# speechcatcher-asr/speechcatcher

Hardware: AMD Instinct MI355X
Metric: concurrent real-time streams (audio-seconds/s), de_xl dims, 640 ms (10240-sample) chunk steps, beam 10 CTC+attention (higher is better)
Workload: dtype f32

## Files before the change

include/scasr.h:

```cpp
#ifndef SCASR_H
#define SCASR_H

#include <stddef.h>
#include <stdint.h>

#ifdef __cplusplus
extern "C" {
#endif

#define SC_OK 0
#define SC_ERR_ARG (-1)
#define SC_ERR_LAUNCH (-2)
#define SC_ERR_CAPACITY (-3)
#define SC_ERR_INPUT (-4)

#define SC_GEMM_RELU 1
#define SC_GEMM_RESIDUAL 2
#define SC_GEMM_LN_AT_CROWS 8
#define SC_GEMM_NAIVE 4
#define SC_GEMM_SPLIT16 16

#define SC_F_ANY_EOS 1
#define SC_F_BEST_EOS 2
#define SC_F_ALL_EOS 4
// ... 351 lines not shown
int sc_ctc_extend_state(const sc_search *sb , void *stream);
int sc_dec_embed(const sc_search *sb, void *stream);
int sc_kv_rows_to_half(const float *stage, const int32_t *rows, int m, int n_layers, int TCAP, int d2,
                       void *ckv_half, void *stream);
int sc_dec_self_attn(const sc_search *sb, int layer, void *stream);
int sc_dec_cross_attn(const sc_search *sb, int layer, void *stream);
int sc_decoder_layers(const sc_search *sb, void *stream);
#define SC_MAX_VOCAB 8192
int sc_logsoftmax_topk(const sc_search *sb, void *stream);
int sc_ctc_prefix_scan(const sc_search *sb, void *stream);
int sc_ctc_prefix_scan_split(const sc_search *sb, int split_min, void *stream);
int sc_fuse_topw(const sc_search *sb, void *stream);
int sc_beam_prune(const sc_search *sb, void *stream);
int sc_ctc_gather_state(const sc_search *sb, void *stream);
int sc_ctc_gather_state_split(const sc_search *sb, int split_min, void *stream);
int sc_decode_step(const sc_search *sb, void *stream);
int sc_decode_step_ex(const sc_search *sb, int scan_split_min, void *stream);
int sc_dec_layer_fused_supported(int d, int H, int W, int F);
int sc_dec_layer_self(const sc_search *sb, int layer, const float *x_in, float *x_out, const float *ffn_part,
                      int n_ffn_part, void *stream);
int sc_dec_layer_cross(const sc_search *sb, int layer, const float *x_in, float *x_out, void *stream);
int sc_dec_layer_ffn(const sc_search *sb, int layer, const float *x_in, float *x_out, float *ffn_part,
                     int max_part, int *n_part , void *stream);
int sc_dec_layer_stream_supported(int d, int H, int W, int F);
int sc_dec_layer_stream(const sc_search *sb, int layer, const float *x_in, float *x_out, float *xn_out,
                        const float *ffn_part, int n_ffn_part, void *stream);
int sc_dec_layer_ffn_xn(const sc_search *sb, int layer, const float *xn, float *ffn_part, int max_part,
                        int *n_part , void *stream);
int sc_dec_layer_reduce_ln(const sc_search *sb, int layer, const float *x_in, float *x_out, float *xn_out, void *stream);
int sc_dec_output_logits(const sc_search *sb, const float *x_in, float *x_out, const float *ffn_part,
// ... 126 lines not shown
```

speechcatcher_amd/_abi.py:

```python
import ctypes as C
import os
import subprocess
from pathlib import Path

HERE = Path(__file__).resolve().parent
LIB_PATH = HERE / "libscasr.so"
CSRC = HERE / "csrc"

c_float_p = C.POINTER(C.c_float)
c_int_p = C.POINTER(C.c_int32)
c_double_p = C.POINTER(C.c_double)
vp = C.c_void_p


class EncLayer(C.Structure):
    _fields_ = [(n, vp) for n in ("ln1_g", "ln1_b", "wqkv", "bqkv", "wo", "bo",
                                  "ln2_g", "ln2_b", "w1", "b1", "w2", "b2", "w1_p", "w2_p",
                                  "wqkv_p", "wo_p", "w1_h", "w2_h", "wqkv_h", "wo_h", "w1_s", "w2_s",
                                  "wqkv_s", "wo_s")]


class DecLayer(C.Structure):
    _fields_ = [(n, vp) for n in ("ln1_g", "ln1_b", "wqkv", "bqkv", "wo", "bo",
                                  "ln2_g", "ln2_b", "wq", "bq", "wo2", "bo2",
# ... 181 lines not shown
    "sc_relpos_attention": (C.c_int, [vp, vp, vp, vp, vp, C.c_int, C.c_int, C.c_int, C.c_int, vp]),
    "sc_relpos_attention_masked": (C.c_int, [vp, vp, vp, vp, vp, C.c_int, C.c_int, C.c_int, C.c_int, vp, C.c_int, vp]),
    "sc_ctc_extend_state": (C.c_int, [vp, vp]),
    "sc_dec_embed": (C.c_int, [vp, vp]),
    "sc_kv_rows_to_half": (C.c_int, [vp, vp, C.c_int, C.c_int, C.c_int, C.c_int, vp, vp]),
    "sc_dec_self_attn": (C.c_int, [vp, C.c_int, vp]),
    "sc_dec_cross_attn": (C.c_int, [vp, C.c_int, vp]),
    "sc_decoder_layers": (C.c_int, [vp, vp]),
    "sc_logsoftmax_topk": (C.c_int, [vp, vp]),
    "sc_ctc_prefix_scan": (C.c_int, [vp, vp]),
    "sc_fuse_topw": (C.c_int, [vp, vp]),
    "sc_beam_prune": (C.c_int, [vp, vp]),
    "sc_ctc_gather_state": (C.c_int, [vp, vp]),
    "sc_ctc_gather_state_split": (C.c_int, [vp, C.c_int, vp]),
    "sc_decode_step": (C.c_int, [vp, vp]),
    "sc_decode_step_ex": (C.c_int, [vp, C.c_int, vp]),
    "sc_ctc_prefix_scan_split": (C.c_int, [vp, C.c_int, vp]),
    "sc_dec_layer_fused_supported": (C.c_int, [C.c_int, C.c_int, C.c_int, C.c_int]),
    "sc_dec_layer_self": (C.c_int, [vp, C.c_int, vp, vp, vp, C.c_int, vp]),
    "sc_dec_layer_cross": (C.c_int, [vp, C.c_int, vp, vp, vp]),
    "sc_dec_layer_ffn": (C.c_int, [vp, C.c_int, vp, vp, vp, C.c_int, C.POINTER(C.c_int), vp]),
    "sc_dec_output_logits": (C.c_int, [vp, vp, vp, vp, C.c_int, vp]),
    "sc_streams_kv_rows": (C.c_int, [vp]),
    "sc_dec_layer_stream_supported": (C.c_int, [C.c_int, C.c_int, C.c_int, C.c_int]),
    "sc_dec_layer_stream": (C.c_int, [vp, C.c_int, vp, vp, vp, vp, C.c_int, vp]),
    "sc_dec_layer_reduce_ln": (C.c_int, [vp, C.c_int, vp, vp, vp, vp]),
    "sc_dec_layer_ffn_xn": (C.c_int, [vp, C.c_int, vp, vp, C.c_int, C.POINTER(C.c_int), vp]),
    "sc_engine_create": (C.c_int, [C.POINTER(Config), C.POINTER(NamedTensor), C.c_int, C.c_int, C.POINTER(vp)]),
    "sc_engine_load": (C.c_int, [C.c_char_p, C.c_int, C.POINTER(vp)]),
    "sc_engine_config": (C.c_int, [vp, C.POINTER(Config)]),
# ... 125 lines not shown
```

speechcatcher_amd/csrc/search.hip:

```cpp
#include "common.h"
#include "attn.h"
#include <mutex>
#include <unordered_map>

#define CTRL(s, f) sb.ctrl[(s) * 8 + (f)]
#define SC_CTC_T(s) (CTRL(s, SC_C_TCTC) > 0 ? CTRL(s, SC_C_TCTC) : CTRL(s, SC_C_T))

#define YSEQ(pp, s, h) (sb.yseq + (((long)(pp) * sb.S + (s)) * sb.W + (h)) * sb.LCAP)
#define XPOS(pp, s, h) (sb.xpos + (((long)(pp) * sb.S + (s)) * sb.W + (h)) * sb.LCAP)
#define ANC(pp, s) (sb.anc + ((long)(pp) * sb.S + (s)) * sb.LCAP * sb.W)
#define CTCR(pp, s) (sb.ctc_r + ((long)(pp) * sb.S + (s)) * sb.TCAP * 2 * sb.W)
#define CTCRS(pp, s) (sb.ctc_rs + ((long)(pp) * sb.S + (s)) * sb.TCAP * sb.W)

__global__ void ctc_extend_state_kernel(sc_search sb) {
  const int s = blockIdx.x, h = threadIdx.x;
  if (!CTRL(s, SC_C_ACTIVE) || !CTRL(s, SC_C_HAS)) return;
  const int T = CTRL(s, SC_C_T), told = CTRL(s, SC_C_TOLD), nh = CTRL(s, SC_C_NHYP);
  if (h >= nh || told >= T) return;
  float *r = CTCR(CTRL(s, SC_C_CUR), s);
  float *rs = CTCRS(CTRL(s, SC_C_CUR), s);
  const float *x = sb.ctcx + (long)s * sb.TCAP * sb.V;
  const int t0 = told < 1 ? 1 : told;
  float rb = r[((long)(t0 - 1) * 2 + 1) * sb.W + h];
  for (int t = t0; t < T; ++t) {
// ... 474 lines not shown
  else {
    const size_t lds = pow2_keys_bytes(sbp->V);
    const int rc = allow_large_lds(reinterpret_cast<const void *>(&logsoftmax_topk_sort_kernel), lds,
                                   pow2_keys_bytes(SC_MAX_VOCAB), "sc_logsoftmax_topk");
    if (rc != SC_OK) return rc;
    logsoftmax_topk_sort_kernel<<<sbp->S * sbp->W, 256, lds, (hipStream_t)stream>>>(*sbp);
  }
  SC_CHECK_LAUNCH();
  return SC_OK;
}

struct CtcChunkT {
  float4 xc[4], xb[4];
  float pn[16], pb[16];
};
#define SC_CTC_CK 16
__host__ __device__ static inline int ctc_tck(int TCAP) { return (TCAP + SC_CTC_CK - 1) / SC_CTC_CK; }
__device__ __forceinline__ void ctc_frame(float &r_n, float &r_b, float prs, float pb, bool same, float xc, float xb, float &phi) {
  phi = same ? pb : prs;
  const float nr_n = lse2(r_n, phi) + xc;
  const float nr_b = lse2(r_n, r_b) + xb;
  r_n = nr_n;
  r_b = nr_b;
}
__device__ __forceinline__ void ctc_psi_add(float &pm, float &ps, float v) {
  const float d = v - pm;
  const float e = sc_exp_neg(-fabsf(d));
  ps = d > 0.f ? ps * e + 1.f : ps + e;
  pm = sc_max_raw(pm, v);
}
__device__ __forceinline__ bool ctc_scan_is_split(int T, int L, int split_min) {
  const int out_len = L - 1;
  int start = out_len > 1 ? out_len : 1;
  if (start > T) start = T;
  return split_min > 0 && T - start >= split_min;
}
#define CTC_NSEG 32
static inline int ctc_split_min_ok(int TCAP, int split_min) { return ctc_tck(TCAP) >= CTC_NSEG ? split_min : 0; }

__global__ __launch_bounds__(256) void ctc_prefix_scan_colmajor_kernel(sc_search sb, int split_min) {
  const int s = blockIdx.y;
  if (!CTRL(s, SC_C_ACTIVE)) return;
  const int nh = CTRL(s, SC_C_NHYP), K = sb.K, W = sb.W, V = sb.V;
  const int e = blockIdx.x * 256 + threadIdx.x;
  if (e >= nh * K) return;
  const int h = e / K, k = e % K;
  const int T = SC_CTC_T(s), L = CTRL(s, SC_C_L), cur = CTRL(s, SC_C_CUR);
  if (ctc_scan_is_split(T, L, split_min)) return;
  const bool has = CTRL(s, SC_C_HAS);
  const long row = (long)s * W + h;
  const int c = sb.pre_ids[row * K + k];
  const int last = YSEQ(cur, s, h)[L - 1];
  const bool same = (c == last);
  const int tct = sb.tct;
  const float *__restrict__ xcol = sb.ctcxT + ((long)s * V + c) * tct;
  const float *__restrict__ xblk = sb.ctcxT + ((long)s * V + sb.blank) * tct;
  const float *__restrict__ rp = CTCR(cur, s);
  const float *__restrict__ rsp = CTCRS(cur, s);
  float *rn = sb.ctc_rnew + (long)s * ctc_tck(sb.TCAP) * 2 * (W * K);
  const int WK = W * K;
  const int out_len = L - 1;
  int start = out_len > 1 ? out_len : 1;
  if (start > T) start = T;
  for (int j = 0; SC_CTC_CK * j + SC_CTC_CK - 1 < start - 1; ++j) {
    rn[((long)j * 2) * WK + e] = SC_LOGZERO;
    rn[((long)j * 2 + 1) * WK + e] = SC_LOGZERO;
  }
  float r_n = (out_len == 0) ? xcol[0] : SC_LOGZERO;
  float r_b = SC_LOGZERO;
  if (((start - 1) & (SC_CTC_CK - 1)) == SC_CTC_CK - 1) {
    rn[((long)((start - 1) / SC_CTC_CK) * 2) * WK + e] = r_n;
    rn[((long)((start - 1) / SC_CTC_CK) * 2 + 1) * WK + e] = r_b;
  }
  float cum = 0.f;
  if (!has)
    for (int t = 0; t < start; ++t) cum += xblk[t];

  auto fetch = [&](CtcChunkT &q, int tb) {
#pragma unroll
    for (int j = 0; j < 4; ++j) {
      const int t4 = min(tb + 4 * j, tct - 4);
      q.xc[j] = *reinterpret_cast<const float4 *>(xcol + t4);
      q.xb[j] = *reinterpret_cast<const float4 *>(xblk + t4);
    }
    if (has) {
#pragma unroll
      for (int i = 0; i < 16; ++i) {
        int t = tb + i;
        t = t < T ? (t < 1 ? 1 : t) : T - 1;
        q.pn[i] = rsp[(long)(t - 1) * W + h];
        q.pb[i] = rp[((long)(t - 1) * 2 + 1) * W + h];
      }
    }
  };
  float pm = r_n, ps = 1.f;
  auto frame = [&](const CtcChunkT &q, int tb, int i) {
    const int t = tb + i;
    const float4 c4 = q.xc[i >> 2], b4 = q.xb[i >> 2];
    const float xc = (i & 3) == 0 ? c4.x : (i & 3) == 1 ? c4.y : (i & 3) == 2 ? c4.z : c4.w;
    const float xb = (i & 3) == 0 ? b4.x : (i & 3) == 1 ? b4.y : (i & 3) == 2 ? b4.z : b4.w;
    const float prs = has ? q.pn[i] : cum;
    const float pb = has ? q.pb[i] : cum;
    float phi;
    ctc_frame(r_n, r_b, prs, pb, same, xc, xb, phi);
    if ((i & (SC_CTC_CK - 1)) == SC_CTC_CK - 1) {
      rn[((long)(t / SC_CTC_CK) * 2) * WK + e] = r_n;
      rn[((long)(t / SC_CTC_CK) * 2 + 1) * WK + e] = r_b;
    }
    ctc_psi_add(pm, ps, phi + xc);
    if (!has) cum += xb;
  };
  auto advance = [&](const CtcChunkT &q, int tb) {
    if (tb >= start && tb + 16 <= T) {
#pragma unroll
      for (int i = 0; i < 16; ++i) frame(q, tb, i);
    } else {
#pragma unroll
      for (int i = 0; i < 16; ++i)
        if (tb + i >= start && tb + i < T) frame(q, tb, i);
    }
  };
  if (start < T) {
    CtcChunkT qa, qb;
    int tb = start & ~15;
    fetch(qa, tb);
    while (true) {
      if (tb + 16 < T) fetch(qb, tb + 16);
      advance(qa, tb);
      tb += 16;
      if (tb >= T) break;
      if (tb + 16 < T) fetch(qa, tb + 16);
      advance(qb, tb);
      tb += 16;
      if (tb >= T) break;
    }
  }
  float psi = pm + logf(ps);
  const float rsum_last = has ? rsp[(long)(T - 1) * W + h] : cum;
  if (c == sb.eos) psi = rsum_last;
  if (c == sb.blank) psi = SC_LOGZERO;
  sb.psi[row * K + k] = psi;
  if (k == 0) sb.psi_eos[row] = rsum_last;
}

#define CTC_EB (256 / CTC_NSEG)
__global__ __launch_bounds__(256) void ctc_prefix_scan_tpar_kernel(sc_search sb, int split_min) {
  __shared__ float co[8][CTC_NSEG][CTC_EB];
  __shared__ float st0[2][CTC_NSEG][CTC_EB];
  __shared__ float cum0[CTC_NSEG][CTC_EB];
  const int s = blockIdx.y;
  if (!CTRL(s, SC_C_ACTIVE)) return;
// ... 143 lines not shown
  std::lock_guard<std::mutex> lk(g_scan_split_mutex);
  g_scan_split[sbp->ctc_rnew] = eff;
}
static int scan_split_last(const sc_search *sbp) {
  std::lock_guard<std::mutex> lk(g_scan_split_mutex);
  auto it = g_scan_split.find(sbp->ctc_rnew);
  return it == g_scan_split.end() ? -1 : it->second;
}

extern "C" int sc_ctc_prefix_scan_split(const sc_search *sbp, int split_min, void *stream) {
  SC_CHECK_ARG(sbp, "null");
  SC_CHECK_ARG(sbp->ctcxT && sbp->tct >= 4 && sbp->tct % 4 == 0, "the prefix scan needs the column-major table copy (sc_search.ctcxT)");
  split_min = ctc_split_min_ok(sbp->TCAP, split_min);
  scan_split_note(sbp, split_min);
  dim3 grid(cdiv(sbp->W * sbp->K, 256), sbp->S);
  ctc_prefix_scan_colmajor_kernel<<<grid, 256, 0, (hipStream_t)stream>>>(*sbp, split_min);
  if (split_min > 0)
    ctc_prefix_scan_tpar_kernel<<<dim3(cdiv(sbp->W * sbp->K, CTC_EB), sbp->S), 256, 0, (hipStream_t)stream>>>(*sbp, split_min);
  SC_CHECK_LAUNCH();
  return SC_OK;
}

extern "C" int sc_ctc_prefix_scan(const sc_search *sbp, void *stream) { return sc_ctc_prefix_scan_split(sbp, 0, stream); }

__device__ __forceinline__ float sort_key_value(unsigned long long c) {
  unsigned u = (unsigned)(c >> 32);
  u = (u & 0x80000000u) ? (u & 0x7FFFFFFFu) : ~u;
  return __uint_as_float(u);
}

__global__ __launch_bounds__(256) void fuse_topw_kernel(sc_search sb) {
  extern __shared__ __attribute__((aligned(16))) float smem[];
  __shared__ int need_full;
  const int row = blockIdx.x, s = row / sb.W, h = row % sb.W;
  if (!CTRL(s, SC_C_ACTIVE) || h >= CTRL(s, SC_C_NHYP)) return;
  const int V = sb.V, K = sb.K, W = sb.W, tid = threadIdx.x;
  float *comb = smem, *ctc = smem + V;
  if (!(sb.w_ctc > 0.f)) {
    if (tid < W) {
      const int c = sb.pre_ids[(long)row * K + tid];
      sb.cand_tok[(long)row * W + tid] = c;
      sb.cand_score[(long)row * W + tid] = __fmul_rn(sb.w_dec, sb.logp[(long)row * V + c]);
      sb.cand_ctc[(long)row * W + tid] = 0.f;
    }
    return;
  }
  const float s_prev = CTRL(s, SC_C_HAS) ? sb.ctc_s[((long)CTRL(s, SC_C_CUR) * sb.S + s) * W + h] : 0.f;
  if (K < 64 && W <= 64 && sb.w_dec >= 0.f) {
    if (tid < 64) {
      const int lane = tid;
      int c = -1;
      float ps = SC_LOGZERO;
      if (lane < K) {
        c = sb.pre_ids[(long)row * K + lane];
        ps = sb.psi[(long)row * K + lane];
      }
      const bool eos_listed = __ballot(c == sb.eos) != 0ull;
      if (lane == K && !eos_listed) c = sb.eos;
      if (c == sb.eos) ps = sb.psi_eos[row];
      if (c == sb.blank) ps = SC_LOGZERO;
      unsigned long long key = 0ull;
      if (c >= 0) {
        const float cv = __fsub_rn(ps, s_prev);
        ctc[c] = cv;
        key = sort_key(__fadd_rn(__fmul_rn(sb.w_dec, sb.logp[(long)row * V + c]), __fmul_rn(sb.w_ctc, cv)), c);
      }
      key = wave_sort64_desc(key, lane);
      const float bound = __fmul_rn(sb.w_ctc, __fsub_rn(SC_LOGZERO, s_prev));
      const unsigned long long kw = shfl_u64(key, W - 1);
      const bool ok = kw != 0ull && sort_key_value(kw) > bound;
      if (lane == 0) need_full = ok ? 0 : 1;
      if (ok && lane < W) {
        const int i = sort_key_index(key);
        sb.cand_tok[(long)row * W + lane] = i;
        sb.cand_score[(long)row * W + lane] = sort_key_value(key);
        sb.cand_ctc[(long)row * W + lane] = ctc[i];
      }
    }
    __syncthreads();
    if (!need_full) return;
    __syncthreads();
  }
  for (int v = tid; v < V; v += 256) ctc[v] = SC_LOGZERO;
  __syncthreads();
  for (int k = tid; k < K; k += 256) ctc[sb.pre_ids[(long)row * K + k]] = sb.psi[(long)row * K + k];
  __syncthreads();
  if (tid == 0) {
    ctc[sb.eos] = sb.psi_eos[row];
    ctc[sb.blank] = SC_LOGZERO;
  }
  __syncthreads();
  for (int v = tid; v < V; v += 256) {
    const float cv = __fsub_rn(ctc[v], s_prev);
    ctc[v] = cv;
    comb[v] = __fadd_rn(__fmul_rn(sb.w_dec, sb.logp[(long)row * V + v]), __fmul_rn(sb.w_ctc, cv));
  }
  __syncthreads();
  const int NP = next_pow2(V);
  unsigned long long *comp = reinterpret_cast<unsigned long long *>(smem + 2 * V);
  for (int c = tid; c < NP; c += 256) comp[c] = c < V ? sort_key(comb[c], c) : 0ull;
  __syncthreads();
  block_bitonic_sort_desc(comp, NP);
  for (int k = tid; k < W; k += 256) {
    const int i = sort_key_index(comp[k]);
    sb.cand_tok[(long)row * W + k] = i;
    sb.cand_score[(long)row * W + k] = comb[i];
    sb.cand_ctc[(long)row * W + k] = ctc[i];
  }
}

extern "C" int sc_fuse_topw(const sc_search *sbp, void *stream) {
  SC_CHECK_ARG(sbp, "null");
  SC_CHECK_ARG(sbp->V > 0 && sbp->V <= SC_MAX_VOCAB, "vocabulary larger than SC_MAX_VOCAB (8192)");
  const size_t smem = fuse_topw_lds(sbp->V);
  const int rc = allow_large_lds(reinterpret_cast<const void *>(&fuse_topw_kernel), smem, fuse_topw_lds(SC_MAX_VOCAB),
                                 "sc_fuse_topw");
  if (rc != SC_OK) return rc;
  fuse_topw_kernel<<<sbp->S * sbp->W, 256, smem, (hipStream_t)stream>>>(*sbp);
  SC_CHECK_LAUNCH();
  return SC_OK;
}

__global__ __launch_bounds__(256) void beam_prune_kernel(sc_search sb) {
  extern __shared__ __attribute__((aligned(16))) double tot[];
  __shared__ int fl_any, fl_all, fl_best, fl_rep;
  __shared__ int win_h[64], win_tok[64];
  __shared__ unsigned bm[SC_KV_MAX_ROWS / 32];
  const int s = blockIdx.x, tid = threadIdx.x;
  if (!CTRL(s, SC_C_ACTIVE)) return;
  for (int w = tid; w < (sb.kv_rows + 31) / 32; w += 256) bm[w] = 0u;
  const int W = sb.W, K = sb.K;
  const int nh = CTRL(s, SC_C_NHYP), L = CTRL(s, SC_C_L), T = CTRL(s, SC_C_T);
  const int cur = CTRL(s, SC_C_CUR), o = 1 - cur;
  const int n = nh * W, nout = n < W ? n : W;
  if (tid == 0) { fl_any = 0; fl_all = 1; fl_best = 0; fl_rep = 0; }
  for (int e = tid; e < n; e += 256) {
    const int h = e / W, j = e % W;
    tot[e] = sb.score[((long)cur * sb.S + s) * W + h] + (double)sb.cand_score[((long)s * W + h) * W + j];
  }
  __syncthreads();
  for (int e = tid; e < n; e += 256) {
    const double te = tot[e];
    int rk = 0;
    for (int j = 0; j < n; ++j) rk += (tot[j] > te) || (tot[j] == te && j < e);
    if (rk >= nout) continue;
    const int h = e / W, j = e % W, i = rk;
    const long prow = (long)s * W + h;
    const int tok = sb.cand_tok[prow * W + j];
    win_h[i] = h;
    win_tok[i] = tok;
    const long oi = ((long)o * sb.S + s) * W + i, ci = ((long)cur * sb.S + s) * W + h;
    sb.score[oi] = te;
    sb.sc_dec[oi] = sb.sc_dec[ci] + (double)sb.logp[prow * sb.V + tok];
    sb.sc_ctc[oi] = sb.sc_ctc[ci] + (double)sb.cand_ctc[prow * W + j];
    int kk = -1;
    for (int q = 0; q < K; ++q)
// ... 5 lines not shown
    else sval = SC_LOGZERO;
    sb.ctc_s[oi] = sval;
    sb.sel[((long)s * W + i) * 2] = h;
    sb.sel[((long)s * W + i) * 2 + 1] = kk < 0 ? 0 : kk;
    const bool is_eos = tok == sb.eos;
    if (is_eos) atomicOr(&fl_any, 1);
    else atomicAnd(&fl_all, 0);
    if (i == 0 && is_eos) atomicOr(&fl_best, 1);
  }
  __syncthreads();
  const int *asrc = ANC(cur, s);
  int *adst = ANC(o, s);
  bool rep = false;
  constexpr int UB = 4;
  const int ntot = nout * (L + 1);
  for (int e0 = tid; e0 < ntot; e0 += 256 * UB) {
    int yv[UB], xv[UB], av[UB];
#pragma unroll
    for (int u = 0; u < UB; ++u) {
      const int e = min(e0 + 256 * u, ntot - 1);
      const int i = e / (L + 1), p = min(e % (L + 1), L - 1);
      const int h = win_h[i];
      yv[u] = YSEQ(cur, s, h)[p];
      xv[u] = XPOS(cur, s, h)[p];
      av[u] = asrc[(long)p * W + h];
    }
#pragma unroll
    for (int u = 0; u < UB; ++u) {
      const int e = e0 + 256 * u;
      if (e >= ntot) break;
      const int i = e / (L + 1), p = e % (L + 1);
      const int tok = win_tok[i];
      int *ydst = YSEQ(o, s, i), *xdst = XPOS(o, s, i);
      if (p < L) {
        ydst[p] = yv[u];
        xdst[p] = xv[u];
        if (p >= 1 && yv[u] == tok && tok != sb.sos && tok != sb.eos) rep = true;
        adst[(long)p * W + i] = av[u];
        atomicOr(&bm[(av[u] >> 5) & (SC_KV_MAX_ROWS / 32 - 1)], 1u << (av[u] & 31));
      } else {
        ydst[L] = tok;
        xdst[L] = T - 1;
      }
    }
// ... 18 lines not shown
      const int t = __shfl_up(incl, o2, 64);
      if (lane >= o2) incl += t;
    }
    int k = got + incl - c;
    while (fr && k < nout) {
      const int b = __ffs(fr) - 1;
      fr &= fr - 1u;
      out[k++] = w * 32 + b;
    }
    got += __shfl(incl, 63, 64);
  }
  if (got < nout && lane >= got && lane < nout) out[lane] = NR - 1;
  if (lane == 0 && sb.kvflags) sb.kvflags[s] = got < nout ? 1 : 0;
}

extern "C" int sc_beam_prune(const sc_search *sbp, void *stream) {
  SC_CHECK_ARG(sbp, "null");
  SC_CHECK_ARG(sbp->W <= 64, "beam wider than 64");
  SC_CHECK_ARG(sbp->kv_rows >= sbp->W && sbp->kv_rows <= SC_KV_MAX_ROWS, "kv_rows out of range (beam .. 65536)");
  size_t smem = (size_t)sbp->W * sbp->W * sizeof(double);
  beam_prune_kernel<<<sbp->S, 256, smem, (hipStream_t)stream>>>(*sbp);
  SC_CHECK_LAUNCH();
  return SC_OK;
}

__global__ __launch_bounds__(256) void ctc_gather_state_kernel(sc_search sb, int split_min) {
  const int s = blockIdx.y;
  if (!CTRL(s, SC_C_ACTIVE)) return;
  const int W = sb.W, K = sb.K, V = sb.V, T = SC_CTC_T(s), nh = CTRL(s, SC_C_NHYP), L = CTRL(s, SC_C_L);
  const int nout = nh * W < W ? nh * W : W;
  const int cur = CTRL(s, SC_C_CUR), o = 1 - cur;
  const bool has = CTRL(s, SC_C_HAS);
  const int WK = W * K, tct = sb.tct;
  float *dst = CTCR(o, s);
  float *dst_rs = CTCRS(o, s);
  const float *__restrict__ rp = CTCR(cur, s);
  const float *__restrict__ rsp = CTCRS(cur, s);
  const float *ck = sb.ctc_rnew + (long)s * ctc_tck(sb.TCAP) * 2 * WK;
  const int out_len = L - 1;
  int start = out_len > 1 ? out_len : 1;
  if (start > T) start = T;
  const bool split = ctc_scan_is_split(T, L, split_min);
  const int base = start & ~15;
  const int seg = split ? 16 * cdiv(T - base, 16 * CTC_NSEG) : SC_CTC_CK;
  const int nseg = split ? CTC_NSEG : cdiv(T, SC_CTC_CK);
  for (int idx = blockIdx.x * blockDim.x + threadIdx.x; idx < nout * nseg; idx += gridDim.x * blockDim.x) {
    const int i = idx % nout, j = idx / nout;
    const int h = sb.sel[((long)s * W + i) * 2], k = sb.sel[((long)s * W + i) * 2 + 1];
    const int e = h * K + k;
    const int c = sb.pre_ids[((long)s * W + h) * K + k];
    const bool same = c == YSEQ(cur, s, h)[L - 1];
    const float *__restrict__ xcol = sb.ctcxT + ((long)s * V + c) * tct;
    const float *__restrict__ xblk = sb.ctcxT + ((long)s * V + sb.blank) * tct;
    int t_lo, t_hi;
    float r_n, r_b;
    if (split) {
      t_lo = max(start, base + j * seg);
      t_hi = min(T, base + (j + 1) * seg);
      r_n = ck[((long)j * 2) * WK + e];
      r_b = ck[((long)j * 2 + 1) * WK + e];
      if (j == 0) {
// ... 52 lines not shown
      for (int q = 0; q < SC_CTC_CK; ++q) {
        const int t = tb + q;
        if (t >= t_lo && t < t_hi) {
          float phi;
          ctc_frame(r_n, r_b, has ? pn[q] : cum, has ? pb[q] : cum, same, xc[q], xb[q], phi);
          dst[((long)t * 2) * W + i] = r_n;
          dst[((long)t * 2 + 1) * W + i] = r_b;
          dst_rs[(long)t * W + i] = lse2(r_n, r_b);
          if (!has) cum += xb[q];
        }
      }
    }
  }
}

extern "C" int sc_ctc_gather_state_split(const sc_search *sbp, int split_min, void *stream) {
  SC_CHECK_ARG(sbp, "null");
  SC_CHECK_ARG(sbp->ctcxT && sbp->tct >= 4, "the state rebuild needs the column-major table copy (sc_search.ctcxT)");
  int gx = cdiv(ctc_tck(sbp->TCAP) * sbp->W, 256);
  if (gx > 16) gx = 16;
  const int eff = ctc_split_min_ok(sbp->TCAP, split_min), last = scan_split_last(sbp);
  if (last >= 0 && last != eff) {
    sc_set_error("sc_ctc_gather_state_split: the last prefix scan of this batch ran with split_min = %d, the rebuild was asked for %d - "
                 "streams split over T leave segment states, not checkpoints: pass the scan's value (sc_ctc_gather_state() = 0)", last, eff);
    return SC_ERR_ARG;
  }
  ctc_gather_state_kernel<<<dim3(gx, sbp->S), 256, 0, (hipStream_t)stream>>>(*sbp, eff);
  SC_CHECK_LAUNCH();
  return SC_OK;
}

extern "C" int sc_ctc_gather_state(const sc_search *sbp, void *stream) { return sc_ctc_gather_state_split(sbp, 0, stream); }

static bool dec_fused_ok(const sc_search &sb) {
  if (const char *e = sc_hook("SC_DEC_FUSED"))
    return atoi(e) != 0 && sc_dec_layer_fused_supported(sb.d, sb.H, sb.W, sb.F) && sb.ph1 && sb.out_w_q;
  if (const char *e = sc_hook("SC_FUSED_MAX"))
    if ((sb.rowmap ? sb.n_rows : sb.S * sb.W) > atoi(e) && sc_dec_layer_hpw(sb) < 2) return false;
  return sc_dec_layer_fused_supported(sb.d, sb.H, sb.W, sb.F) && sb.ph1 && sb.ph2 && sb.ffn_part &&
         sb.max_ffn_part >= 1 && sb.out_w_q && sb.V % sb.d == 0 && sb.layers && sb.layers[0].wqkv_pp &&
         sb.layers[0].wq_pp && sb.layers[0].wo_pp && sb.layers[0].w1_p;
}

int sc_decode_step_form(const sc_search *sbp) { return dec_fused_ok(*sbp) ? (sc_dec_layer_stream_form(*sbp) ? 2 : 1) : 0; }

extern "C" int sc_decode_step(const sc_search *sbp, void *stream) { return sc_decode_step_ex(sbp, 0, stream); }

// ... 23 lines not shown
      } else
      SC_TRY(sc_dec_layer_ffn(sbp, li, xa, xb, sb.ffn_part, sb.max_ffn_part, &npart, stream));
      float *t = xa; xa = xb; xb = t;
    }
    SC_TRY(sc_dec_output_logits(sbp, xa, xb, sb.ffn_part, npart, stream));
  } else {
  SC_TRY(sc_dec_embed(sbp, stream));
  bool logits_done = false;
  SC_TRY(decoder_layers_impl(sbp, stream, true, &logits_done));
  if (!logits_done)
    SC_TRY(sc_gemm(sb.dxn, sb.rowmap, sb.d, sb.out_w, sb.out_b, sb.logits, sb.rowmap, sb.V, n, sb.V, sb.d, 0, 0, stream));
  }
  SC_TRY(sc_logsoftmax_topk(sbp, stream));
  const bool use_ctc = sb.w_ctc > 0.f;
  if (use_ctc) SC_TRY(sc_ctc_prefix_scan_split(sbp, scan_split_min, stream));
  SC_TRY(sc_fuse_topw(sbp, stream));
  SC_TRY(sc_beam_prune(sbp, stream));
  if (use_ctc) SC_TRY(sc_ctc_gather_state_split(sbp, scan_split_min, stream));
  return SC_OK;
}
```

speechcatcher_amd/hip_backend.py:

```python
import ctypes as C
import os
import warnings

import torch

from . import _abi


def _p(t):
    return 0 if t is None else t.data_ptr()


def resample(x, rate, device="cuda:0"):
    if not torch.cuda.is_available():
        raise _abi.ScasrError("resample needs a ROCm GPU (torch.cuda.is_available() is False)")
    lib = _abi.load()
    device = torch.device(device)
    x = torch.as_tensor(x).to(device, torch.float32).contiguous().reshape(-1)
    n_out = int(lib.sc_resample_out_count(int(rate), x.numel(), 1))
    if n_out < 0:
        _abi.check(n_out, "sc_resample_out_count")
    y = torch.empty(n_out, dtype=torch.float32, device=device)
    with torch.cuda.device(device):
        n = int(lib.sc_resample(_p(x), x.numel(), int(rate), _p(y), n_out, torch.cuda.current_stream(device).cuda_stream))
# ... 582 lines not shown
    def logsoftmax_topk(self, sb):
        self._sb_call("sc_logsoftmax_topk", sb)

    def ctc_prefix_scan(self, sb, split_min=0):
        self._sb_call("sc_ctc_prefix_scan_split", sb, int(split_min))

    def fuse_topw(self, sb):
        self._sb_call("sc_fuse_topw", sb)

    def beam_prune(self, sb):
        self._sb_call("sc_beam_prune", sb)

    def ctc_gather_state(self, sb, split_min=0):
        self._sb_call("sc_ctc_gather_state_split", sb, int(split_min))

    def decode_step(self, sb):
        if not self.use_graphs:
            self._sb_call("sc_decode_step", sb)
            return
        graphs = getattr(sb, "_sc_decode_graphs", None)
        if graphs is None:
            graphs = sb._sc_decode_graphs = {}
        g = graphs.get(int(sb.n_rows_step))
        st = self._stream()
        if g is None:
            if st == 0:
                raise _abi.ScasrError("hipGraph capture needs a non-default stream (StreamBatch.stream)")
            self._sb_call("sc_decode_step", sb)
            self._chk(self.lib.sc_graph_capture_begin(st), "sc_graph_capture_begin")
            try:
# ... 22 lines not shown
```

Measured before the change: 4050.

## Fuse candidate fusion and beam prune into one per-stream tail kernel; stage CTC scan rows in LDS

Adds a search tail kernel that runs the per-row fast top-W fusion, any full-vocabulary fallback, and beam pruning within one 1024-thread workgroup per stream. This replaces two separate launches and the global round trip of candidates between them. Separately, the CTC prefix scan now stages the shared blank column and the per-hypothesis previous-state rows in double-buffered LDS with a three-deep register prefetch, instead of each thread loading them redundantly from global memory. In exchange the scan adds block barriers and the tail runs one large workgroup per stream, which may limit parallelism when there are few streams.

```diff
diff --git a/include/scasr.h b/include/scasr.h
--- a/include/scasr.h
+++ b/include/scasr.h
@@ -389,6 +389,7 @@
 int sc_beam_prune(const sc_search *sb, void *stream);
 int sc_ctc_gather_state(const sc_search *sb, void *stream);
 int sc_ctc_gather_state_split(const sc_search *sb, int split_min, void *stream);
+int sc_search_tail(const sc_search *sb, int split_min, void *stream);
 int sc_decode_step(const sc_search *sb, void *stream);
 int sc_decode_step_ex(const sc_search *sb, int scan_split_min, void *stream);
 int sc_dec_layer_fused_supported(int d, int H, int W, int F);
diff --git a/speechcatcher_amd/_abi.py b/speechcatcher_amd/_abi.py
--- a/speechcatcher_amd/_abi.py
+++ b/speechcatcher_amd/_abi.py
@@ -219,6 +219,7 @@
     "sc_ctc_gather_state": (C.c_int, [vp, vp]),
     "sc_ctc_gather_state_split": (C.c_int, [vp, C.c_int, vp]),
     "sc_decode_step": (C.c_int, [vp, vp]),
+    "sc_search_tail": (C.c_int, [vp, C.c_int, vp]),
     "sc_decode_step_ex": (C.c_int, [vp, C.c_int, vp]),
     "sc_ctc_prefix_scan_split": (C.c_int, [vp, C.c_int, vp]),
     "sc_dec_layer_fused_supported": (C.c_int, [C.c_int, C.c_int, C.c_int, C.c_int]),
diff --git a/speechcatcher_amd/csrc/search.hip b/speechcatcher_amd/csrc/search.hip
--- a/speechcatcher_amd/csrc/search.hip
+++ b/speechcatcher_amd/csrc/search.hip
@@ -512,6 +512,9 @@
   float4 xc[4], xb[4];
   float pn[16], pb[16];
 };
+#define CTC_STG_ROW 32
+__host__ __device__ static inline int ctc_scan_rows_cap(int W, int K) { const int r = 255 / K + 2; return r < W ? r : W; }
+__host__ __device__ static inline int ctc_scan_stage_floats(int W, int K) { return 16 + CTC_STG_ROW * ctc_scan_rows_cap(W, K); }
 #define SC_CTC_CK 16
 __host__ __device__ static inline int ctc_tck(int TCAP) { return (TCAP + SC_CTC_CK - 1) / SC_CTC_CK; }
 __device__ __forceinline__ void ctc_frame(float &r_n, float &r_b, float prs, float pb, bool same, float xc, float xb, float &phi) {
@@ -536,15 +539,21 @@
 #define CTC_NSEG 32
 static inline int ctc_split_min_ok(int TCAP, int split_min) { return ctc_tck(TCAP) >= CTC_NSEG ? split_min : 0; }
 
+template <int NST>
 __global__ __launch_bounds__(256) void ctc_prefix_scan_colmajor_kernel(sc_search sb, int split_min) {
+  extern __shared__ __attribute__((aligned(16))) float stg[];
   const int s = blockIdx.y;
   if (!CTRL(s, SC_C_ACTIVE)) return;
   const int nh = CTRL(s, SC_C_NHYP), K = sb.K, W = sb.W, V = sb.V;
-  const int e = blockIdx.x * 256 + threadIdx.x;
-  if (e >= nh * K) return;
-  const int h = e / K, k = e % K;
+  const int e0 = blockIdx.x * 256, tid = threadIdx.x;
+  if (e0 >= nh * K) return;
   const int T = SC_CTC_T(s), L = CTRL(s, SC_C_L), cur = CTRL(s, SC_C_CUR);
   if (ctc_scan_is_split(T, L, split_min)) return;
+  const bool live = e0 + tid < nh * K;
+  const int e = live ? e0 + tid : nh * K - 1;
+  const int h = e / K, k = e % K;
+  const int h_lo = e0 / K, nrow = min((e0 + 255) / K, nh - 1) - h_lo + 1;
+  const int sfl = ctc_scan_stage_floats(W, K);
   const bool has = CTRL(s, SC_C_HAS);
   const long row = (long)s * W + h;
   const int c = sb.pre_ids[row * K + k];
@@ -560,13 +569,14 @@
   const int out_len = L - 1;
   int start = out_len > 1 ? out_len : 1;
   if (start > T) start = T;
-  for (int j = 0; SC_CTC_CK * j + SC_CTC_CK - 1 < start - 1; ++j) {
-    rn[((long)j * 2) * WK + e] = SC_LOGZERO;
-    rn[((long)j * 2 + 1) * WK + e] = SC_LOGZERO;
-  }
+  if (live)
+    for (int j = 0; SC_CTC_CK * j + SC_CTC_CK - 1 < start - 1; ++j) {
+      rn[((long)j * 2) * WK + e] = SC_LOGZERO;
+      rn[((long)j * 2 + 1) * WK + e] = SC_LOGZERO;
+    }
   float r_n = (out_len == 0) ? xcol[0] : SC_LOGZERO;
   float r_b = SC_LOGZERO;
-  if (((start - 1) & (SC_CTC_CK - 1)) == SC_CTC_CK - 1) {
+  if (live && ((start - 1) & (SC_CTC_CK - 1)) == SC_CTC_CK - 1) {
     rn[((long)((start - 1) / SC_CTC_CK) * 2) * WK + e] = r_n;
     rn[((long)((start - 1) / SC_CTC_CK) * 2 + 1) * WK + e] = r_b;
   }
@@ -574,65 +584,101 @@
   if (!has)
     for (int t = 0; t < start; ++t) cum += xblk[t];
 
-  auto fetch = [&](CtcChunkT &q, int tb) {
-#pragma unroll
-    for (int j = 0; j < 4; ++j) {
-      const int t4 = min(tb + 4 * j, tct - 4);
-      q.xc[j] = *reinterpret_cast<const float4 *>(xcol + t4);
-      q.xb[j] = *reinterpret_cast<const float4 *>(xblk + t4);
-    }
-    if (has) {
-#pragma unroll
-      for (int i = 0; i < 16; ++i) {
+  auto stage_load = [&](float (&sv)[NST], int tb) {
+#pragma unroll
+    for (int u = 0; u < NST; ++u) {
+      const int idx = tid + 256 * u;
+      if (idx < 16) {
+        sv[u] = xblk[min(tb + (idx & ~3), tct - 4) + (idx & 3)];
+      } else if (has && idx - 16 < nrow * CTC_STG_ROW) {
+        const int r = (idx - 16) / CTC_STG_ROW, i = idx & 15;
+        const bool second = ((idx - 16) & 16) != 0;
         int t = tb + i;
         t = t < T ? (t < 1 ? 1 : t) : T - 1;
-        q.pn[i] = rsp[(long)(t - 1) * W + h];
-        q.pb[i] = rp[((long)(t - 1) * 2 + 1) * W + h];
+        sv[u] = second ? rp[((long)(t - 1) * 2 + 1) * W + h_lo + r] : rsp[(long)(t - 1) * W + h_lo + r];
       }
     }
+  };
+  auto stage_store = [&](const float (&sv)[NST], int buf) {
+#pragma unroll
+    for (int u = 0; u < NST; ++u) {
+      const int idx = tid + 256 * u;
+      if (idx < 16 || (has && idx - 16 < nrow * CTC_STG_ROW)) stg[buf * sfl + idx] = sv[u];
+    }
+  };
+  auto fetch = [&](float4 (&q)[4], int tb) {
+#pragma unroll
+    for (int j = 0; j < 4; ++j) q[j] = *reinterpret_cast<const float4 *>(xcol + min(tb + 4 * j, tct - 4));
   };
   float pm = r_n, ps = 1.f;
-  auto frame = [&](const CtcChunkT &q, int tb, int i) {
-    const int t = tb + i;
-    const float4 c4 = q.xc[i >> 2], b4 = q.xb[i >> 2];
-    const float xc = (i & 3) == 0 ? c4.x : (i & 3) == 1 ? c4.y : (i & 3) == 2 ? c4.z : c4.w;
-    const float xb = (i & 3) == 0 ? b4.x : (i & 3) == 1 ? b4.y : (i & 3) == 2 ? b4.z : b4.w;
-    const float prs = has ? q.pn[i] : cum;
-    const float pb = has ? q.pb[i] : cum;
-    float phi;
-    ctc_frame(r_n, r_b, prs, pb, same, xc, xb, phi);
-    if ((i & (SC_CTC_CK - 1)) == SC_CTC_CK - 1) {
-      rn[((long)(t / SC_CTC_CK) * 2) * WK + e] = r_n;
-      rn[((long)(t / SC_CTC_CK) * 2 + 1) * WK + e] = r_b;
-    }
-    ctc_psi_add(pm, ps, phi + xc);
-    if (!has) cum += xb;
-  };
-  auto advance = [&](const CtcChunkT &q, int tb) {
+  auto advance = [&](const float4 (&q)[4], int tb, int buf) {
+    const float4 *sp = reinterpret_cast<const float4 *>(stg + buf * sfl);
+    const float4 *hp = sp + 4 + (h - h_lo) * (CTC_STG_ROW / 4);
+    float4 xb4[4], pn4[4] = {}, pb4[4] = {};
+#pragma unroll
+    for (int j = 0; j < 4; ++j) xb4[j] = sp[j];
+    if (has) {
+#pragma unroll
+      for (int j = 0; j < 4; ++j) {
+        pn4[j] = hp[j];
+        pb4[j] = hp[4 + j];
+      }
+    }
+    auto frame = [&](int i) {
+      const int t = tb + i;
+      const float4 c4 = q[i >> 2], b4 = xb4[i >> 2], n4 = pn4[i >> 2], p4 = pb4[i >> 2];
+      const float xc = (i & 3) == 0 ? c4.x : (i & 3) == 1 ? c4.y : (i & 3) == 2 ? c4.z : c4.w;
+      const float xb = (i & 3) == 0 ? b4.x : (i & 3) == 1 ? b4.y : (i & 3) == 2 ? b4.z : b4.w;
+      const float qn = (i & 3) == 0 ? n4.x : (i & 3) == 1 ? n4.y : (i & 3) == 2 ? n4.z : n4.w;
+      const float qb = (i & 3) == 0 ? p4.x : (i & 3) == 1 ? p4.y : (i & 3) == 2 ? p4.z : p4.w;
+      const float prs = has ? qn : cum;
+      const float pb = has ? qb : cum;
+      float phi;
+      ctc_frame(r_n, r_b, prs, pb, same, xc, xb, phi);
+      if (live && (i & (SC_CTC_CK - 1)) == SC_CTC_CK - 1) {
+        rn[((long)(t / SC_CTC_CK) * 2) * WK + e] = r_n;
+        rn[((long)(t / SC_CTC_CK) * 2 + 1) * WK + e] = r_b;
+      }
+      ctc_psi_add(pm, ps, phi + xc);
+      if (!has) cum += xb;
+    };
     if (tb >= start && tb + 16 <= T) {
 #pragma unroll
-      for (int i = 0; i < 16; ++i) frame(q, tb, i);
+      for (int i = 0; i < 16; ++i) frame(i);
     } else {
 #pragma unroll
       for (int i = 0; i < 16; ++i)
-        if (tb + i >= start && tb + i < T) frame(q, tb, i);
+        if (tb + i >= start && tb + i < T) frame(i);
     }
   };
   if (start < T) {
-    CtcChunkT qa, qb;
-    int tb = start & ~15;
+    float sv[NST];
+    float4 qa[4], qb[4], qc[4];
+    int tb = start & ~15, buf = 0;
+    stage_load(sv, tb);
     fetch(qa, tb);
+    if (tb + 16 < T) fetch(qb, tb + 16);
+    if (tb + 32 < T) fetch(qc, tb + 32);
+    stage_store(sv, 0);
+    if (tb + 16 < T) stage_load(sv, tb + 16);
+    __syncthreads();
+#define CTC_SCAN_STEP(Q)                                   \
+    advance(Q, tb, buf);                                   \
+    if (tb + 16 < T) stage_store(sv, buf ^ 1);             \
+    if (tb + 32 < T) stage_load(sv, tb + 32);              \
+    if (tb + 48 < T) fetch(Q, tb + 48);                    \
+    __syncthreads();                                       \
+    tb += 16;                                              \
+    buf ^= 1;                                              \
+    if (tb >= T) break;
     while (true) {
-      if (tb + 16 < T) fetch(qb, tb + 16);
-      advance(qa, tb);
-      tb += 16;
-      if (tb >= T) break;
-      if (tb + 16 < T) fetch(qa, tb + 16);
-      advance(qb, tb);
-      tb += 16;
-      if (tb >= T) break;
-    }
-  }
+      CTC_SCAN_STEP(qa)
+      CTC_SCAN_STEP(qb)
+      CTC_SCAN_STEP(qc)
+    }
+#undef CTC_SCAN_STEP
+  }
+  if (!live) return;
   float psi = pm + logf(ps);
   const float rsum_last = has ? rsp[(long)(T - 1) * W + h] : cum;
   if (c == sb.eos) psi = rsum_last;
@@ -806,7 +852,13 @@
   split_min = ctc_split_min_ok(sbp->TCAP, split_min);
   scan_split_note(sbp, split_min);
   dim3 grid(cdiv(sbp->W * sbp->K, 256), sbp->S);
-  ctc_prefix_scan_colmajor_kernel<<<grid, 256, 0, (hipStream_t)stream>>>(*sbp, split_min);
+  const int sfl = ctc_scan_stage_floats(sbp->W, sbp->K);
+  SC_CHECK_ARG(sbp->K > 0 && sfl <= 9 * 256, "the prefix scan stages at most 64 hypothesis rows per workgroup (beam <= 64)");
+  const size_t lds = 2 * (size_t)sfl * sizeof(float);
+  if (sfl <= 2 * 256)
+    ctc_prefix_scan_colmajor_kernel<2><<<grid, 256, lds, (hipStream_t)stream>>>(*sbp, split_min);
+  else
+    ctc_prefix_scan_colmajor_kernel<9><<<grid, 256, lds, (hipStream_t)stream>>>(*sbp, split_min);
   if (split_min > 0)
     ctc_prefix_scan_tpar_kernel<<<dim3(cdiv(sbp->W * sbp->K, CTC_EB), sbp->S), 256, 0, (hipStream_t)stream>>>(*sbp, split_min);
   SC_CHECK_LAUNCH();
@@ -819,6 +871,80 @@
   unsigned u = (unsigned)(c >> 32);
   u = (u & 0x80000000u) ? (u & 0x7FFFFFFFu) : ~u;
   return __uint_as_float(u);
+}
+
+__device__ __forceinline__ void fuse_row_dec_only(const sc_search &sb, int row, int tid) {
+  const int V = sb.V, K = sb.K, W = sb.W;
+  if (tid < W) {
+    const int c = sb.pre_ids[(long)row * K + tid];
+    sb.cand_tok[(long)row * W + tid] = c;
+    sb.cand_score[(long)row * W + tid] = __fmul_rn(sb.w_dec, sb.logp[(long)row * V + c]);
+    sb.cand_ctc[(long)row * W + tid] = 0.f;
+  }
+}
+__device__ __forceinline__ float fuse_row_s_prev(const sc_search &sb, int s, int h) {
+  return CTRL(s, SC_C_HAS) ? sb.ctc_s[((long)CTRL(s, SC_C_CUR) * sb.S + s) * sb.W + h] : 0.f;
+}
+__device__ __forceinline__ bool fuse_fast_ok(const sc_search &sb) { return sb.K < 64 && sb.W <= 64 && sb.w_dec >= 0.f; }
+__device__ __forceinline__ bool fuse_row_fast(const sc_search &sb, int row, float s_prev, int lane, float *ctc) {
+  const int V = sb.V, K = sb.K, W = sb.W;
+  int c = -1;
+  float ps = SC_LOGZERO;
+  if (lane < K) {
+    c = sb.pre_ids[(long)row * K + lane];
+    ps = sb.psi[(long)row * K + lane];
+  }
+  const bool eos_listed = __ballot(c == sb.eos) != 0ull;
+  if (lane == K && !eos_listed) c = sb.eos;
+  if (c == sb.eos) ps = sb.psi_eos[row];
+  if (c == sb.blank) ps = SC_LOGZERO;
+  unsigned long long key = 0ull;
+  if (c >= 0) {
+    const float cv = __fsub_rn(ps, s_prev);
+    ctc[c] = cv;
+    key = sort_key(__fadd_rn(__fmul_rn(sb.w_dec, sb.logp[(long)row * V + c]), __fmul_rn(sb.w_ctc, cv)), c);
+  }
+  key = wave_sort64_desc(key, lane);
+  const float bound = __fmul_rn(sb.w_ctc, __fsub_rn(SC_LOGZERO, s_prev));
+  const unsigned long long kw = shfl_u64(key, W - 1);
+  const bool ok = kw != 0ull && sort_key_value(kw) > bound;
+  if (ok && lane < W) {
+    const int i = sort_key_index(key);
+    sb.cand_tok[(long)row * W + lane] = i;
+    sb.cand_score[(long)row * W + lane] = sort_key_value(key);
+    sb.cand_ctc[(long)row * W + lane] = ctc[i];
+  }
+  return ok;
+}
+__device__ __forceinline__ void fuse_row_full(const sc_search &sb, int row, float s_prev, int tid, int nthr, float *smem) {
+  const int V = sb.V, K = sb.K, W = sb.W;
+  float *comb = smem, *ctc = smem + V;
+  for (int v = tid; v < V; v += nthr) ctc[v] = SC_LOGZERO;
+  __syncthreads();
+  for (int k = tid; k < K; k += nthr) ctc[sb.pre_ids[(long)row * K + k]] = sb.psi[(long)row * K + k];
+  __syncthreads();
+  if (tid == 0) {
+    ctc[sb.eos] = sb.psi_eos[row];
+    ctc[sb.blank] = SC_LOGZERO;
+  }
+  __syncthreads();
+  for (int v = tid; v < V; v += nthr) {
+    const float cv = __fsub_rn(ctc[v], s_prev);
+    ctc[v] = cv;
+    comb[v] = __fadd_rn(__fmul_rn(sb.w_dec, sb.logp[(long)row * V + v]), __fmul_rn(sb.w_ctc, cv));
+  }
+  __syncthreads();
+  const int NP = next_pow2(V);
+  unsigned long long *comp = reinterpret_cast<unsigned long long *>(smem + 2 * V);
+  for (int c = tid; c < NP; c += nthr) comp[c] = c < V ? sort_key(comb[c], c) : 0ull;
+  __syncthreads();
+  block_bitonic_sort_desc(comp, NP);
+  for (int k = tid; k < W; k += nthr) {
+    const int i = sort_key_index(comp[k]);
+    sb.cand_tok[(long)row * W + k] = i;
+    sb.cand_score[(long)row * W + k] = comb[i];
+    sb.cand_ctc[(long)row * W + k] = ctc[i];
+  }
 }
 
 __global__ __launch_bounds__(256) void fuse_topw_kernel(sc_search sb) {
@@ -826,79 +952,22 @@
   __shared__ int need_full;
   const int row = blockIdx.x, s = row / sb.W, h = row % sb.W;
   if (!CTRL(s, SC_C_ACTIVE) || h >= CTRL(s, SC_C_NHYP)) return;
-  const int V = sb.V, K = sb.K, W = sb.W, tid = threadIdx.x;
-  float *comb = smem, *ctc = smem + V;
+  const int tid = threadIdx.x;
   if (!(sb.w_ctc > 0.f)) {
-    if (tid < W) {
-      const int c = sb.pre_ids[(long)row * K + tid];
-      sb.cand_tok[(long)row * W + tid] = c;
-      sb.cand_score[(long)row * W + tid] = __fmul_rn(sb.w_dec, sb.logp[(long)row * V + c]);
-      sb.cand_ctc[(long)row * W + tid] = 0.f;
-    }
+    fuse_row_dec_only(sb, row, tid);
     return;
   }
-  const float s_prev = CTRL(s, SC_C_HAS) ? sb.ctc_s[((long)CTRL(s, SC_C_CUR) * sb.S + s) * W + h] : 0.f;
-  if (K < 64 && W <= 64 && sb.w_dec >= 0.f) {
+  const float s_prev = fuse_row_s_prev(sb, s, h);
+  if (fuse_fast_ok(sb)) {
     if (tid < 64) {
-      const int lane = tid;
-      int c = -1;
-      float ps = SC_LOGZERO;
-      if (lane < K) {
-        c = sb.pre_ids[(long)row * K + lane];
-        ps = sb.psi[(long)row * K + lane];
-      }
-      const bool eos_listed = __ballot(c == sb.eos) != 0ull;
-      if (lane == K && !eos_listed) c = sb.eos;
-      if (c == sb.eos) ps = sb.psi_eos[row];
-      if (c == sb.blank) ps = SC_LOGZERO;
-      unsigned long long key = 0ull;
-      if (c >= 0) {
-        const float cv = __fsub_rn(ps, s_prev);
-        ctc[c] = cv;
-        key = sort_key(__fadd_rn(__fmul_rn(sb.w_dec, sb.logp[(long)row * V + c]), __fmul_rn(sb.w_ctc, cv)), c);
-      }
-      key = wave_sort64_desc(key, lane);
-      const float bound = __fmul_rn(sb.w_ctc, __fsub_rn(SC_LOGZERO, s_prev));
-      const unsigned long long kw = shfl_u64(key, W - 1);
-      const bool ok = kw != 0ull && sort_key_value(kw) > bound;
-      if (lane == 0) need_full = ok ? 0 : 1;
-      if (ok && lane < W) {
-        const int i = sort_key_index(key);
-        sb.cand_tok[(long)row * W + lane] = i;
-        sb.cand_score[(long)row * W + lane] = sort_key_value(key);
-        sb.cand_ctc[(long)row * W + lane] = ctc[i];
-      }
+      const bool ok = fuse_row_fast(sb, row, s_prev, tid, smem + sb.V);
+      if (tid == 0) need_full = ok ? 0 : 1;
     }
     __syncthreads();
     if (!need_full) return;
     __syncthreads();
   }
-  for (int v = tid; v < V; v += 256) ctc[v] = SC_LOGZERO;
-  __syncthreads();
-  for (int k = tid; k < K; k += 256) ctc[sb.pre_ids[(long)row * K + k]] = sb.psi[(long)row * K + k];
-  __syncthreads();
-  if (tid == 0) {
-    ctc[sb.eos] = sb.psi_eos[row];
-    ctc[sb.blank] = SC_LOGZERO;
-  }
-  __syncthreads();
-  for (int v = tid; v < V; v += 256) {
-    const float cv = __fsub_rn(ctc[v], s_prev);
-    ctc[v] = cv;
-    comb[v] = __fadd_rn(__fmul_rn(sb.w_dec, sb.logp[(long)row * V + v]), __fmul_rn(sb.w_ctc, cv));
-  }
-  __syncthreads();
-  const int NP = next_pow2(V);
-  unsigned long long *comp = reinterpret_cast<unsigned long long *>(smem + 2 * V);
-  for (int c = tid; c < NP; c += 256) comp[c] = c < V ? sort_key(comb[c], c) : 0ull;
-  __syncthreads();
-  block_bitonic_sort_desc(comp, NP);
-  for (int k = tid; k < W; k += 256) {
-    const int i = sort_key_index(comp[k]);
-    sb.cand_tok[(long)row * W + k] = i;
-    sb.cand_score[(long)row * W + k] = comb[i];
-    sb.cand_ctc[(long)row * W + k] = ctc[i];
-  }
+  fuse_row_full(sb, row, s_prev, tid, 256, smem);
 }
 
 extern "C" int sc_fuse_topw(const sc_search *sbp, void *stream) {
@@ -913,25 +982,22 @@
   return SC_OK;
 }
 
-__global__ __launch_bounds__(256) void beam_prune_kernel(sc_search sb) {
-  extern __shared__ __attribute__((aligned(16))) double tot[];
+__device__ __forceinline__ void beam_prune_stream(const sc_search &sb, int s, int tid, int nthr, double *tot) {
   __shared__ int fl_any, fl_all, fl_best, fl_rep;
   __shared__ int win_h[64], win_tok[64];
   __shared__ unsigned bm[SC_KV_MAX_ROWS / 32];
-  const int s = blockIdx.x, tid = threadIdx.x;
-  if (!CTRL(s, SC_C_ACTIVE)) return;
-  for (int w = tid; w < (sb.kv_rows + 31) / 32; w += 256) bm[w] = 0u;
+  for (int w = tid; w < (sb.kv_rows + 31) / 32; w += nthr) bm[w] = 0u;
   const int W = sb.W, K = sb.K;
   const int nh = CTRL(s, SC_C_NHYP), L = CTRL(s, SC_C_L), T = CTRL(s, SC_C_T);
   const int cur = CTRL(s, SC_C_CUR), o = 1 - cur;
   const int n = nh * W, nout = n < W ? n : W;
   if (tid == 0) { fl_any = 0; fl_all = 1; fl_best = 0; fl_rep = 0; }
-  for (int e = tid; e < n; e += 256) {
+  for (int e = tid; e < n; e += nthr) {
     const int h = e / W, j = e % W;
     tot[e] = sb.score[((long)cur * sb.S + s) * W + h] + (double)sb.cand_score[((long)s * W + h) * W + j];
   }
   __syncthreads();
-  for (int e = tid; e < n; e += 256) {
+  for (int e = tid; e < n; e += nthr) {
     const double te = tot[e];
     int rk = 0;
     for (int j = 0; j < n; ++j) rk += (tot[j] > te) || (tot[j] == te && j < e);
@@ -967,11 +1033,11 @@
   bool rep = false;
   constexpr int UB = 4;
   const int ntot = nout * (L + 1);
-  for (int e0 = tid; e0 < ntot; e0 += 256 * UB) {
+  for (int e0 = tid; e0 < ntot; e0 += nthr * UB) {
     int yv[UB], xv[UB], av[UB];
 #pragma unroll
     for (int u = 0; u < UB; ++u) {
-      const int e = min(e0 + 256 * u, ntot - 1);
+      const int e = min(e0 + nthr * u, ntot - 1);
       const int i = e / (L + 1), p = min(e % (L + 1), L - 1);
       const int h = win_h[i];
       yv[u] = YSEQ(cur, s, h)[p];
@@ -980,7 +1046,7 @@
     }
 #pragma unroll
     for (int u = 0; u < UB; ++u) {
-      const int e = e0 + 256 * u;
+      const int e = e0 + nthr * u;
       if (e >= ntot) break;
       const int i = e / (L + 1), p = e % (L + 1);
       const int tok = win_tok[i];
@@ -1029,6 +1095,13 @@
   if (lane == 0 && sb.kvflags) sb.kvflags[s] = got < nout ? 1 : 0;
 }
 
+__global__ __launch_bounds__(256) void beam_prune_kernel(sc_search sb) {
+  extern __shared__ __attribute__((aligned(16))) double tot[];
+  const int s = blockIdx.x;
+  if (!CTRL(s, SC_C_ACTIVE)) return;
+  beam_prune_stream(sb, s, threadIdx.x, 256, tot);
+}
+
 extern "C" int sc_beam_prune(const sc_search *sbp, void *stream) {
   SC_CHECK_ARG(sbp, "null");
   SC_CHECK_ARG(sbp->W <= 64, "beam wider than 64");
@@ -1039,9 +1112,7 @@
   return SC_OK;
 }
 
-__global__ __launch_bounds__(256) void ctc_gather_state_kernel(sc_search sb, int split_min) {
-  const int s = blockIdx.y;
-  if (!CTRL(s, SC_C_ACTIVE)) return;
+__device__ __forceinline__ void ctc_gather_state_stream(const sc_search &sb, int s, int split_min, int idx0, int stride) {
   const int W = sb.W, K = sb.K, V = sb.V, T = SC_CTC_T(s), nh = CTRL(s, SC_C_NHYP), L = CTRL(s, SC_C_L);
   const int nout = nh * W < W ? nh * W : W;
   const int cur = CTRL(s, SC_C_CUR), o = 1 - cur;
@@ -1059,7 +1130,7 @@
   const int base = start & ~15;
   const int seg = split ? 16 * cdiv(T - base, 16 * CTC_NSEG) : SC_CTC_CK;
   const int nseg = split ? CTC_NSEG : cdiv(T, SC_CTC_CK);
-  for (int idx = blockIdx.x * blockDim.x + threadIdx.x; idx < nout * nseg; idx += gridDim.x * blockDim.x) {
+  for (int idx = idx0; idx < nout * nseg; idx += stride) {
     const int i = idx % nout, j = idx / nout;
     const int h = sb.sel[((long)s * W + i) * 2], k = sb.sel[((long)s * W + i) * 2 + 1];
     const int e = h * K + k;
@@ -1142,6 +1213,12 @@
   }
 }
 
+__global__ __launch_bounds__(256) void ctc_gather_state_kernel(sc_search sb, int split_min) {
+  const int s = blockIdx.y;
+  if (!CTRL(s, SC_C_ACTIVE)) return;
+  ctc_gather_state_stream(sb, s, split_min, blockIdx.x * blockDim.x + threadIdx.x, gridDim.x * blockDim.x);
+}
+
 extern "C" int sc_ctc_gather_state_split(const sc_search *sbp, int split_min, void *stream) {
   SC_CHECK_ARG(sbp, "null");
   SC_CHECK_ARG(sbp->ctcxT && sbp->tct >= 4, "the state rebuild needs the column-major table copy (sc_search.ctcxT)");
@@ -1159,6 +1236,65 @@
 }
 
 extern "C" int sc_ctc_gather_state(const sc_search *sbp, void *stream) { return sc_ctc_gather_state_split(sbp, 0, stream); }
+
+#define SC_TAIL_THREADS 1024
+static size_t search_tail_tot_bytes(int W) { return (((size_t)W * W * sizeof(double)) + 15) & ~(size_t)15; }
+static size_t search_tail_lds(int W, int V) {
+  const int nw = W < SC_TAIL_THREADS / 64 ? W : SC_TAIL_THREADS / 64;
+  const size_t fast = (size_t)nw * V * sizeof(float), full = fuse_topw_lds(V);
+  return search_tail_tot_bytes(W) + (fast > full ? fast : full);
+}
+#define SC_TAIL_MAX_LDS (128 * 1024)
+
+__global__ __launch_bounds__(SC_TAIL_THREADS) void search_tail_kernel(sc_search sb, int tot_bytes) {
+  extern __shared__ __attribute__((aligned(16))) unsigned char tail_lds[];
+  __shared__ int need_full[64];
+  const int s = blockIdx.x, tid = threadIdx.x, wave = tid >> 6, lane = tid & 63;
+  if (!CTRL(s, SC_C_ACTIVE)) return;
+  const int W = sb.W, V = sb.V, nh = CTRL(s, SC_C_NHYP);
+  double *tot = reinterpret_cast<double *>(tail_lds);
+  float *fl = reinterpret_cast<float *>(tail_lds + tot_bytes);
+  const bool use_ctc = sb.w_ctc > 0.f;
+  for (int h = wave; h < nh; h += SC_TAIL_THREADS / 64) {
+    const int row = s * W + h;
+    int nf = 0;
+    if (!use_ctc) fuse_row_dec_only(sb, row, lane);
+    else if (!fuse_fast_ok(sb)) nf = 1;
+    else nf = fuse_row_fast(sb, row, fuse_row_s_prev(sb, s, h), lane, fl + (long)wave * V) ? 0 : 1;
+    if (lane == 0) need_full[h] = nf;
+  }
+  __syncthreads();
+  for (int h = 0; h < nh; ++h) {
+    if (!need_full[h]) continue;
+    fuse_row_full(sb, s * W + h, fuse_row_s_prev(sb, s, h), tid, SC_TAIL_THREADS, fl);
+    __syncthreads();
+  }
+  beam_prune_stream(sb, s, tid, SC_TAIL_THREADS, tot);
+}
+
+static bool search_tail_supported(const sc_search &sb) {
+  return sb.W >= 1 && sb.W <= 64 && sb.V > 0 && sb.V <= SC_MAX_VOCAB &&
+         search_tail_lds(sb.W, sb.V) <= SC_TAIL_MAX_LDS;
+}
+
+extern "C" int sc_search_tail(const sc_search *sbp, int split_min, void *stream) {
+  SC_CHECK_ARG(sbp, "null");
+  SC_CHECK_ARG(search_tail_supported(*sbp), "sc_search_tail: beam <= 64 and the vocabulary within SC_MAX_VOCAB");
+  SC_CHECK_ARG(sbp->kv_rows >= sbp->W && sbp->kv_rows <= SC_KV_MAX_ROWS, "kv_rows out of range (beam .. 65536)");
+  const size_t lds = search_tail_lds(sbp->W, sbp->V);
+  const int rc = allow_large_lds(reinterpret_cast<const void *>(&search_tail_kernel), lds + 9 * 1024, SC_TAIL_MAX_LDS, "sc_search_tail");
+  if (rc != SC_OK) return rc;
+  search_tail_kernel<<<sbp->S, SC_TAIL_THREADS, lds, (hipStream_t)stream>>>(*sbp, (int)search_tail_tot_bytes(sbp->W));
+  SC_CHECK_LAUNCH();
+  if (sbp->w_ctc > 0.f) return sc_ctc_gather_state_split(sbp, split_min, stream);
+  return SC_OK;
+}
+
+static bool search_tail_ok(const sc_search &sb) {
+  if (const char *e = sc_hook("SC_SEARCH_TAIL"))
+    if (atoi(e) == 0) return false;
+  return search_tail_supported(sb) && sb.kv_rows >= sb.W && sb.kv_rows <= SC_KV_MAX_ROWS;
+}
 
 static bool dec_fused_ok(const sc_search &sb) {
   if (const char *e = sc_hook("SC_DEC_FUSED"))
@@ -1212,6 +1348,7 @@
   SC_TRY(sc_logsoftmax_topk(sbp, stream));
   const bool use_ctc = sb.w_ctc > 0.f;
   if (use_ctc) SC_TRY(sc_ctc_prefix_scan_split(sbp, scan_split_min, stream));
+  if (search_tail_ok(sb)) return sc_search_tail(sbp, scan_split_min, stream);
   SC_TRY(sc_fuse_topw(sbp, stream));
   SC_TRY(sc_beam_prune(sbp, stream));
   if (use_ctc) SC_TRY(sc_ctc_gather_state_split(sbp, scan_split_min, stream));
diff --git a/speechcatcher_amd/hip_backend.py b/speechcatcher_amd/hip_backend.py
--- a/speechcatcher_amd/hip_backend.py
+++ b/speechcatcher_amd/hip_backend.py
@@ -620,6 +620,9 @@
     def ctc_gather_state(self, sb, split_min=0):
         self._sb_call("sc_ctc_gather_state_split", sb, int(split_min))
 
+    def search_tail(self, sb, split_min=0):
+        self._sb_call("sc_search_tail", sb, int(split_min))
+
     def decode_step(self, sb):
         if not self.use_graphs:
             self._sb_call("sc_decode_step", sb)
```

Result: no change. 4101 (median of 6 runs) (+1.3%).
